# jdm365/Compression_Algorithms

Measured on AMD Instinct MI355X. Metric: encode GB/s on enwik9 at 1/2/4/8 MI355X; ratio vs ref; round-trip bit-exact, higher is better.
Workload: dtype u8; 1 GPU; deflate (LZ77 W=32 KiB len<=31 + per-block dynamic Huffman over the 286-symbol alphabet, mode H), independent 64 KiB blocks; 1000000000 enwik-shaped bytes in the job, 1000000000 on rank 0; input_seed=12345, mode=H, input_bytes_job=1000000000, input_bytes_rank0=1000000000, compressed_bytes_job=516875560, compressed_bytes_rank0=516875560, gather_to_rank0=False, parallelism=blocks sharded over 1 GPU(s), weak scaling

## Files before the change

### compression_algorithms_amd/csrc/common.h

```cpp
#pragma once

#include <hip/hip_runtime.h>
#include <stdint.h>
#include <stdio.h>
#include <string.h>

#include "../../include/mi_codec.h"
#include "lz_plan.h"

#define MI_WAVE 64

#define MI_PROF_KERNELS 48
#define MI_PROF_PENDING 8192
struct mi_prof_entry {
    const char *name;
    double      ms;
    uint64_t    launches, bytes;
};
struct mi_prof_pending { hipEvent_t a, b; uint64_t bytes; int idx; };

struct mi_ctx {
    int         device = 0;
    hipStream_t stream = nullptr;
    hipStream_t side = nullptr;
    hipStream_t fb = nullptr;
    hipStream_t fb2 = nullptr;
    hipStream_t parse = nullptr;
    hipEvent_t  ev_find[MI_SETS] = {}, ev_done[MI_SETS] = {}, ev_part[MI_SETS] = {}, ev_fb[MI_SETS] = {}, ev_replay[MI_SETS] = {}, ev_wide[MI_SETS] = {};
    hipEvent_t  ev_fork = nullptr;
    int         last_hip = 0;
    int         profiling = 0;
    int         num_cu = 256;
    int         lds_rank_ok = 0;
    int         test_break_rank = 0;
    int         test_force_fb = 0;
    int         test_small_parts = 0;
    int         test_old_partition = 0;
    uint64_t   *d_stats = nullptr;
    uint32_t   *h_order = nullptr;
    uint32_t   *d_order = nullptr;
    uint32_t    order_violations = 0;
    uint32_t    order_reported = 0;
    void       *ws = nullptr;
    size_t      ws_bytes = 0;
#ifdef MI_TEST_HOOKS
    size_t      ws_asked = 0;
    const void *test_partmap = nullptr, *test_partmap_meta = nullptr;
    uint32_t    test_partmap_nb = 0;
#endif
    void       *h_pinned = nullptr;
    size_t      h_pinned_bytes = 0;
    uint64_t   *lz_dbg = nullptr;
    uint32_t   *d_err = nullptr;
    uint32_t    err_next = 0;
#define MI_ERR_SLOTS 256
    mi_prof_entry    prof[MI_PROF_KERNELS];
    int              nprof = 0;
    mi_prof_pending *pending = nullptr;
    int              npending = 0;
    hipEvent_t      *event_pool = nullptr;
    int              npool = 0;
};

#define MI_HIP(ctx, call)                                                     \
    do {                                                                      \
        hipError_t e__ = (call);                                              \
        if (e__ != hipSuccess) {                                              \
            (ctx)->last_hip = (int)e__;                                       \
            return MI_ERR_HIP;                                                \
        }                                                                     \
    } while (0)

int mi_order_poll(mi_ctx *ctx);
mi_status mi_ws_reserve(mi_ctx *ctx, size_t bytes);
uint32_t *mi_err_slot(mi_ctx *ctx, hipStream_t s);
extern "C" mi_status mi_validate_block_table(const uint64_t *h_block_bits, uint64_t nblocks, uint64_t stream_bytes, uint32_t align_bits);
hipStream_t mi_host_stream(mi_ctx *ctx);
struct mi_prof_scope {
    mi_ctx *ctx; int idx; hipStream_t s; hipEvent_t a = nullptr, b = nullptr; uint64_t pbytes = 0;
    mi_prof_scope(mi_ctx *c, const char *name, hipStream_t st, uint64_t bytes);
    ~mi_prof_scope();
};

static inline size_t mi_align_up(size_t v, size_t a) { return (v + a - 1) / a * a; }

struct mi_carver {
    uint8_t *base; size_t limit, off = 0; bool overflow = false;
    explicit mi_carver(void *b = nullptr, size_t lim = SIZE_MAX) : base((uint8_t *)b), limit(lim) {}
    template <typename T> T *take(size_t count) {
        const size_t at = mi_align_up(off, 256);
        off = at + count * sizeof(T);
        if (off > limit) overflow = true;
        return base && !overflow ? (T *)(base + at) : nullptr;
    }
    template <typename T> void take(T *&p, size_t count) { p = take<T>(count); }
    template <typename T> static T *at(T *p, size_t i) { return p ? p + i : nullptr; }
    size_t bytes() const { return mi_align_up(off, 256); }
};
template <typename F> static inline mi_status mi_ws_carve(mi_ctx *ctx, F layout)
{
    mi_carver m;
    layout(m);
    const mi_status st = mi_ws_reserve(ctx, m.bytes());
    if (st) return st;
    mi_carver cv(ctx->ws);
    layout(cv);
    return MI_OK;
}
```

### compression_algorithms_amd/csrc/ctx.hip

```cpp
#include "common.h"
#include <stdlib.h>

__global__ __launch_bounds__(512)
static void k_lds_rank_probe(uint32_t rounds, uint32_t *__restrict__ bad)
{
    __shared__ uint32_t cnt[256 * 9];
    const uint32_t tid = threadIdx.x, lane = tid & 63u, wave = tid >> 6;
    for (uint32_t i = tid; i < 256 * 9; i += 512) cnt[i] = 0;
    __syncthreads();
    uint32_t errs = 0, x = tid * 2654435761u + blockIdx.x * 40503u + 12345u;
    for (uint32_t r = 0; r < rounds; ++r) {
        x = x * 1664525u + 1013904223u;
        const uint32_t ndig = 1u << (r % 9u);
        const uint32_t d = (blockIdx.x & 1u) ? ((x >> 16) % ndig) : (((x >> 16) % ndig) * 32u) % 256u;
        const uint32_t old = atomicAdd(&cnt[d * 9 + wave], 1u);
        for (uint32_t o = 1; o < 64; ++o) {
            const uint32_t src = (lane + o) & 63u;
            const uint32_t od = __shfl(d, src), oo = __shfl(old, src);
            if (od == d && ((src < lane) != (oo < old))) ++errs;
        }
    }
    if (errs) atomicAdd(bad, errs);
}

static int lds_rank_selfcheck(mi_ctx *c)
{
    if (getenv("MI_LZ_NO_ARANK")) return 0;
    uint32_t h = 1;
    if (hipMemset(c->d_err, 0, 4) != hipSuccess) return 0;
    hipLaunchKernelGGL(k_lds_rank_probe, dim3(64), dim3(512), 0, 0, 72u, c->d_err);
    if (hipGetLastError() != hipSuccess || hipMemcpy(&h, c->d_err, 4, hipMemcpyDeviceToHost) != hipSuccess) return 0;
    (void)hipMemset(c->d_err, 0, 4);
    return h == 0;
}

extern "C" {

const char *mi_version(void) { return "mi_codec 0.1 (gfx950)"; }

const char *mi_status_str(mi_status s)
{
    switch (s) {
    case MI_OK: return "ok";
    case MI_ERR_ARG: return "bad argument";
    case MI_ERR_HIP: return "HIP call failed";
    case MI_ERR_NOMEM: return "out of memory";
    case MI_ERR_CAPACITY: return "output buffer too small";
    case MI_ERR_EMPTY_INPUT: return "empty input (reference: ERROR: Queue is empty)";
    case MI_ERR_SINGLE_SYMBOL: return "single distinct symbol (reference: ERROR: No code for character)";
    case MI_ERR_CODE_TOO_LONG: return "Huffman code longer than 32 bits";
    case MI_ERR_CORRUPT: return "corrupt stream";
    case MI_ERR_NO_DEVICE: return "no HIP device: this library has no CPU fallback";
    case MI_ERR_TRANSPORT: return "multi-device gather: RCCL missing or an RCCL call failed";
    case MI_ERR_UNSTABLE: return "a sort came out unstable (LDS atomics not lane-ordered): encode again, the context now ranks with ballots";
    }
    return "unknown";
}

mi_status mi_ctx_create(mi_ctx **out, int device)
{
    if (!out) return MI_ERR_ARG;
    *out = nullptr;
    int count = 0;
    if (hipGetDeviceCount(&count) != hipSuccess || count <= 0 || device < 0 || device >= count)
        return MI_ERR_NO_DEVICE;
    mi_ctx *c = (mi_ctx *)calloc(1, sizeof(mi_ctx));
    if (!c) return MI_ERR_NOMEM;
    c->num_cu = 256;
    c->device = device;
    if (hipSetDevice(device) != hipSuccess) { free(c); return MI_ERR_NO_DEVICE; }
    hipDeviceProp_t prop;
    if (hipGetDeviceProperties(&prop, device) == hipSuccess) c->num_cu = prop.multiProcessorCount;
    {
        int lo = 0, hi = 0;
        (void)hipDeviceGetStreamPriorityRange(&lo, &hi);
        bool ok = hipStreamCreateWithFlags(&c->side, hipStreamNonBlocking) == hipSuccess;
        ok = ok && hipStreamCreateWithPriority(&c->fb, hipStreamNonBlocking, lo) == hipSuccess;
        ok = ok && hipStreamCreateWithPriority(&c->parse, hipStreamNonBlocking, hi) == hipSuccess;
        if (!ok) { mi_ctx_destroy(c); return MI_ERR_HIP; }
    }
    for (int i = 0; i < MI_SETS; ++i) {
        hipEventCreateWithFlags(&c->ev_replay[i], hipEventDisableTiming);
        hipEventCreateWithFlags(&c->ev_wide[i], hipEventDisableTiming);
        hipEventCreateWithFlags(&c->ev_part[i], hipEventDisableTiming);
        hipEventCreateWithFlags(&c->ev_fb[i], hipEventDisableTiming);
        hipEventCreateWithFlags(&c->ev_find[i], hipEventDisableTiming);
        hipEventCreateWithFlags(&c->ev_done[i], hipEventDisableTiming);
    }
    hipEventCreateWithFlags(&c->ev_fork, hipEventDisableTiming);
    c->h_pinned_bytes = 1 << 16;
    if (hipHostMalloc(&c->h_pinned, c->h_pinned_bytes, hipHostMallocDefault) != hipSuccess) {
        mi_ctx_destroy(c); return MI_ERR_NOMEM;
    }
    if (hipMalloc((void **)&c->d_err, MI_ERR_SLOTS * sizeof(uint32_t)) != hipSuccess) { mi_ctx_destroy(c); return MI_ERR_NOMEM; }
    if (hipHostMalloc((void **)&c->h_order, 64, hipHostMallocMapped) != hipSuccess ||
        hipHostGetDevicePointer((void **)&c->d_order, c->h_order, 0) != hipSuccess) { mi_ctx_destroy(c); return MI_ERR_NOMEM; }
    c->h_order[0] = 0; c->h_order[1] = 0; c->h_order[2] = 0;
    c->lds_rank_ok = lds_rank_selfcheck(c);
    c->test_break_rank = getenv("MI_LZ_TEST_BREAK_RANK") != nullptr;
    c->test_force_fb = getenv("MI_LZ_TEST_FORCE_FALLBACK") != nullptr;
    c->test_small_parts = getenv("MI_LZ_TEST_SMALL_PARTS") != nullptr;
    c->test_old_partition = getenv("MI_LZ_TEST_OLD_PARTITION") != nullptr;
    if (hipMalloc((void **)&c->d_stats, 64) != hipSuccess || hipMemset(c->d_stats, 0, 64) != hipSuccess) { mi_ctx_destroy(c); return MI_ERR_NOMEM; }
    *out = c;
    return MI_OK;
}

void mi_ctx_destroy(mi_ctx *c)
{
    if (!c) return;
    hipSetDevice(c->device);
    hipDeviceSynchronize();
    for (int i = 0; i < c->npending; ++i) { hipEventDestroy(c->pending[i].a); hipEventDestroy(c->pending[i].b); }
    for (int i = 0; i < c->npool; ++i) hipEventDestroy(c->event_pool[i]);
    free(c->pending); free(c->event_pool);
    if (c->ws) hipFree(c->ws);
    if (c->d_err) hipFree(c->d_err);
    if (c->d_stats) hipFree(c->d_stats);
    if (c->h_pinned) hipHostFree(c->h_pinned);
    if (c->h_order) hipHostFree(c->h_order);
    if (c->stream) hipStreamDestroy(c->stream);
    if (c->side) hipStreamDestroy(c->side);
    if (c->fb) hipStreamDestroy(c->fb);
    if (c->fb2) hipStreamDestroy(c->fb2);
    if (c->parse) hipStreamDestroy(c->parse);
    for (int i = 0; i < MI_SETS; ++i) {
        if (c->ev_replay[i]) hipEventDestroy(c->ev_replay[i]);
        if (c->ev_wide[i]) hipEventDestroy(c->ev_wide[i]);
        if (c->ev_find[i]) hipEventDestroy(c->ev_find[i]);
        if (c->ev_done[i]) hipEventDestroy(c->ev_done[i]);
        if (c->ev_part[i]) hipEventDestroy(c->ev_part[i]);
        if (c->ev_fb[i]) hipEventDestroy(c->ev_fb[i]);
    }
    if (c->ev_fork) hipEventDestroy(c->ev_fork);
    free(c);
}

int mi_last_hip_error(const mi_ctx *c) { return c ? c->last_hip : 0; }

mi_status mi_sync(mi_ctx *c, void *stream)
{
    if (!c) return MI_ERR_ARG;
    MI_HIP(c, hipStreamSynchronize((hipStream_t)stream));
    mi_order_poll(c);
    if (c->order_violations != c->order_reported) { c->order_reported = c->order_violations; return MI_ERR_UNSTABLE; }
    return MI_OK;
}

uint32_t mi_order_violations(mi_ctx *c)
{
    if (!c) return 0;
    mi_order_poll(c);
    return c->order_violations;
}

mi_status mi_lz_path_stats(mi_ctx *c, uint64_t *fallback_blocks, uint64_t *wide_parts)
{
    if (!c || !c->d_stats) return MI_ERR_ARG;
    uint64_t h[2] = {0, 0};
    MI_HIP(c, hipSetDevice(c->device));
    MI_HIP(c, hipDeviceSynchronize());
    MI_HIP(c, hipMemcpy(h, c->d_stats, 16, hipMemcpyDeviceToHost));
    if (fallback_blocks) *fallback_blocks = h[0];
    if (wide_parts) *wide_parts = h[1];
    return MI_OK;
}

mi_status mi_set_profiling(mi_ctx *c, int on)
{
    if (!c) return MI_ERR_ARG;
    if (on && !c->pending) {
        c->pending = (mi_prof_pending *)calloc(MI_PROF_PENDING, sizeof(mi_prof_pending));
        c->event_pool = (hipEvent_t *)calloc(2 * MI_PROF_PENDING, sizeof(hipEvent_t));
        if (!c->pending || !c->event_pool) { free(c->pending); free(c->event_pool); c->pending = nullptr; c->event_pool = nullptr; return MI_ERR_NOMEM; }
    }
    c->profiling = on;
    return MI_OK;
}

int mi_get_kernel_times(mi_ctx *c, mi_kernel_time *out, int cap)
{
    if (!c || !out) return 0;
    for (int i = 0; i < c->npending; ++i) {
        mi_prof_pending &q = c->pending[i];
        float ms = 0.f;
        hipEventSynchronize(q.b);
        if (hipEventElapsedTime(&ms, q.a, q.b) == hipSuccess) {
            mi_prof_entry &p = c->prof[q.idx];
            p.ms += ms; p.launches += 1; p.bytes += q.bytes;
        }
        c->event_pool[c->npool++] = q.a;
        c->event_pool[c->npool++] = q.b;
    }
    c->npending = 0;
    int n = 0;
    for (int i = 0; i < c->nprof; ++i) {
        mi_prof_entry &p = c->prof[i];
        if (!p.launches || n >= cap) continue;
        out[n].name = p.name;
        out[n].ms = p.ms / (double)p.launches;
        out[n].launches = p.launches;
        out[n].bytes = p.bytes;
        ++n;
        p.ms = 0; p.launches = 0; p.bytes = 0;
    }
    return n;
}

}

uint32_t *mi_err_slot(mi_ctx *c, hipStream_t s)
{
    uint32_t *e = c->d_err + (c->err_next++ % MI_ERR_SLOTS);
    if (hipMemsetAsync(e, 0, 4, s) != hipSuccess) return nullptr;
    return e;
}

extern "C" mi_status mi_validate_block_table(const uint64_t *t, uint64_t nblocks, uint64_t stream_bytes, uint32_t align_bits)
{
    if (!t || !align_bits) return MI_ERR_ARG;
    if (stream_bytes > (UINT64_MAX >> 3)) return MI_ERR_ARG;
    const uint64_t limit = stream_bytes * 8;
    uint64_t prev = t[0];
    if (prev % align_bits) return MI_ERR_CORRUPT;
    for (uint64_t i = 1; i <= nblocks; ++i) {
        const uint64_t v = t[i];
        if (v < prev || (v % align_bits)) return MI_ERR_CORRUPT;
        prev = v;
    }
    return prev <= limit ? MI_OK : MI_ERR_CORRUPT;
}

hipStream_t mi_host_stream(mi_ctx *c)
{
    if (!c->stream && hipStreamCreateWithFlags(&c->stream, hipStreamNonBlocking) != hipSuccess) c->stream = nullptr;
    return c->stream;
}


int mi_order_poll(mi_ctx *c)
{
    if (!c->h_order) return 0;
    const uint32_t v = __atomic_exchange_n(c->h_order, 0u, __ATOMIC_RELAXED);
    if (!v) return 0;
    ++c->order_violations;
    c->lds_rank_ok = 0;
    return 1;
}

#ifdef MI_TEST_HOOKS
#define MI_WS_GUARD 4096u
#else
#define MI_WS_GUARD 0u
#endif

mi_status mi_ws_reserve(mi_ctx *c, size_t bytes)
{
#ifdef MI_TEST_HOOKS
    if (bytes > c->ws_asked) c->ws_asked = bytes;
#endif
    if (bytes + MI_WS_GUARD <= c->ws_bytes) return MI_OK;
    MI_HIP(c, hipDeviceSynchronize());
    if (c->ws) { MI_HIP(c, hipFree(c->ws)); c->ws = nullptr; c->ws_bytes = 0; }
    size_t want = mi_align_up(bytes + bytes / 8 + MI_WS_GUARD, 1 << 20);
    if (hipMalloc(&c->ws, want) != hipSuccess) {
        (void)hipGetLastError();
        want = mi_align_up(bytes + MI_WS_GUARD, 1 << 20);
        c->ws = nullptr;
        if (hipMalloc(&c->ws, want) != hipSuccess) { (void)hipGetLastError(); c->ws = nullptr; return MI_ERR_NOMEM; }
    }
    c->ws_bytes = want;
    return MI_OK;
}

#ifdef MI_TEST_HOOKS
extern "C" int64_t mi_test_ws_guard(mi_ctx *c, int op)
{
    if (!c || op < 0 || op > 2) return -2;
    if (op == 0) { c->ws_asked = 0; return -1; }
    if (hipDeviceSynchronize() != hipSuccess) return -2;
    const size_t from = c->ws_asked < c->ws_bytes ? c->ws_asked : c->ws_bytes, len = c->ws_bytes - from;
    uint8_t *d = (uint8_t *)c->ws + from;
    if (op == 1) return !len || hipMemset(d, 0xA5, len) == hipSuccess ? -1 : -2;
    uint8_t *h = (uint8_t *)malloc(len ? len : 1);
    if (!h) return -2;
    int64_t at = -1;
    if (len && hipMemcpy(h, d, len, hipMemcpyDeviceToHost) != hipSuccess) at = -2;
    for (size_t i = 0; at == -1 && i < len; ++i) if (h[i] != 0xA5) at = (int64_t)(from + i);
    free(h);
    return at;
}
#endif

static hipEvent_t take_event(mi_ctx *c)
{
    if (c->npool > 0) return c->event_pool[--c->npool];
    hipEvent_t e = nullptr;
    hipEventCreate(&e);
    return e;
}

mi_prof_scope::mi_prof_scope(mi_ctx *c, const char *name, hipStream_t st, uint64_t bytes) : ctx(c), idx(-1), s(st)
{
    if (!c->profiling || !c->pending || c->npending >= MI_PROF_PENDING) return;
    for (int i = 0; i < c->nprof; ++i) if (strcmp(c->prof[i].name, name) == 0) { idx = i; break; }
    if (idx < 0) {
        if (c->nprof >= MI_PROF_KERNELS) return;
        idx = c->nprof++;
        c->prof[idx].name = name; c->prof[idx].ms = 0; c->prof[idx].launches = 0; c->prof[idx].bytes = 0;
    }
    a = take_event(c); b = take_event(c);
    pbytes = bytes;
    hipEventRecord(a, s);
}

mi_prof_scope::~mi_prof_scope()
{
    if (idx < 0) return;
    hipEventRecord(b, s);
    mi_prof_pending &q = ctx->pending[ctx->npending++];
    q.a = a; q.b = b; q.bytes = pbytes; q.idx = idx;
}
```

### compression_algorithms_amd/csrc/lz2_partition.hip

```cpp
#include "lz_common.h"
#include "lz2.h"
#include "internal.h"

namespace {
#define PT_TICK(k) do { if (sc.dbg && tid == 0) { long long t2 = clock64(); atomicAdd((unsigned long long *)&sc.dbg[32 + (k)], (unsigned long long)(t2 - tk)); tk = t2; } } while (0)

struct Lz2PartLds {
    uint32_t *s_grp;
    uint32_t *s_safe;
    uint64_t *s_scan64;
    uint32_t *s_scan32;
    uint32_t *s_thr;
    uint32_t *s_pstart;
    uint8_t  *s_gpart;
    uint8_t  *s_wrank;
    uint32_t *s_s0, *s_flag;
    uint32_t *s_K, *s_wbase, *s_wbase2;
};

__device__ __forceinline__ bool lz2_partition_cuts(const Lz2PartLds &L, const LzP &P, const Lz2Scratch &sc, uint32_t lb, uint32_t n, int tid, long long &tk,
                                                   uint32_t &gstart_out)
{
    uint32_t *const s_grp = L.s_grp, *const s_safe = L.s_safe, *const s_scan32 = L.s_scan32, *const s_thr = L.s_thr, *const s_pstart = L.s_pstart;
    uint64_t *const s_scan64 = L.s_scan64;
    uint8_t *const s_gpart = L.s_gpart, *const s_wrank = L.s_wrank;
    uint32_t &s_s0 = *L.s_s0, &s_flag = *L.s_flag, &s_K = *L.s_K, &s_wbase = *L.s_wbase, &s_wbase2 = *L.s_wbase2;
    const uint32_t T = 1u << P.tbits;
    const uint32_t gshift = P.tbits - LZ2_NG_BITS, Gw = 1u << gshift;

    const uint32_t g0 = tid * (LZ2_NG / 1024);
    AffMax mine{0, AM_NEG};
    for (uint32_t k = 0; k < LZ2_NG / 1024; ++k) {
        const int32_t c = (int32_t)s_grp[g0 + k];
        mine = am_then(mine, AffMax{c - (int32_t)Gw, c > 0 ? c - 1 : 0});
    }
    uint64_t tot64;
    const uint64_t pre64 = block_exclusive_scan<uint64_t>(am_pack(mine), OpAm(), am_pack(AffMax{0, AM_NEG}), s_scan64, &tot64);
    const AffMax pre = am_unpack(pre64), total = am_unpack(tot64);
    const int32_t x0 = P.deflate ? (total.b > 0 ? total.b : 0) : 0;
    {
        int32_t x = x0 + pre.a > pre.b ? x0 + pre.a : pre.b;
        if (x < 0) x = 0;
        uint32_t safe_bits = 0;
        for (uint32_t k = 0; k < LZ2_NG / 1024; ++k) {
            const int32_t c = (int32_t)s_grp[g0 + k];
            int32_t o = x + c - (int32_t)Gw;
            const int32_t o2 = c > 0 ? c - 1 : 0;
            o = o > o2 ? o : o2;
            if (o < 0) o = 0;
            if (o == 0) safe_bits |= 1u << k;
            x = o;
        }
        atomicOr(&s_safe[g0 >> 5], safe_bits << (g0 & 31u));
        if (safe_bits) atomicMin(&s_s0, g0 + (uint32_t)__builtin_ctz(safe_bits));
    }
    {
        uint32_t sum = 0;
        for (uint32_t k = 0; k < LZ2_NG / 1024; ++k) sum += s_grp[g0 + k];
        uint32_t tot;
        uint32_t run = block_exclusive_scan<uint32_t>(sum, OpAddU32(), 0u, s_scan32, &tot);
        for (uint32_t k = 0; k < LZ2_NG / 1024; ++k) { run += s_grp[g0 + k]; s_grp[g0 + k] = run; }
    }
    __syncthreads();

    PT_TICK(2);
    Lz2BlockMeta *mt = sc.meta + lb;
    const uint32_t s0 = s_s0;
    const bool no_safe = (s0 == ~0u);
    const uint32_t gstart = P.deflate ? (no_safe ? 0u : ((s0 + 1u) & (LZ2_NG - 1u))) : 0u;
    const uint32_t base = gstart << gshift;
    auto cum_incl = [&](uint32_t gr) -> uint32_t {
        const uint32_t g = (gstart + gr) & (LZ2_NG - 1u);
        const uint32_t before = gstart ? s_grp[gstart - 1] : 0u;
        return g >= gstart ? s_grp[g] - before : s_grp[g] + (n - before);
    };
    auto is_safe = [&](uint32_t gr) -> bool {
        const uint32_t g = (gstart + gr) & (LZ2_NG - 1u);
        return (s_safe[g >> 5] >> (g & 31u)) & 1u;
    };
    if (tid < 64) {
        const uint32_t lane = (uint32_t)tid;
        uint32_t k = 0, cur = 0, glo = 0;
        bool bad = false;
        if (lane == 0) s_thr[0] = 0;
        auto cut_below = [&](uint32_t limit) -> int32_t {
            const uint32_t span = (gshift <= 6u) ? (65536u >> gshift) : LZ2_NG;
            uint32_t lo = glo, hi = (glo + span < LZ2_NG) ? glo + span : LZ2_NG - 1;
            while (lo < hi) {
                const uint32_t len = hi - lo, step = (len + 63u) / 64u;
                const uint32_t pr = lo + lane * step;
                const bool over = (pr < hi) && cum_incl(pr) > limit;
                const uint64_t mk = __ballot(over);
                if (mk == 0ull) lo = lo + ((len - 1u) / step) * step + 1u;
                else {
                    const uint32_t j = (uint32_t)__builtin_ctzll(mk);
                    hi = lo + j * step;
                    if (j) lo = lo + (j - 1u) * step + 1u;
                }
            }
            for (int32_t g = (int32_t)lo - 1; g >= (int32_t)glo; g -= 64) {
                const int32_t c = g - (int32_t)lane;
                const uint64_t mk = __ballot(c >= (int32_t)glo && is_safe((uint32_t)c));
                if (mk) return g - (int32_t)__builtin_ctzll(mk);
            }
            return -1;
        };
#ifdef MI_TEST_HOOKS
        const uint32_t cap_s = (P.flags & LZP_SMALL_PARTS) ? 640u : LZ2_CAP_S;
#else
        constexpr uint32_t cap_s = LZ2_CAP_S;
#endif
        while (n - cur > cap_s) {
            int32_t gr = cut_below(cur + cap_s);
            if (gr < (int32_t)glo) {
                if (n - cur <= LZ2_CAP) break;
                gr = cut_below(cur + LZ2_CAP);
            }
            if (gr < (int32_t)glo || k + 2 > LZ2_MAXPARTS) { bad = true; break; }
            cur = cum_incl((uint32_t)gr);
            glo = (uint32_t)gr + 1u;
            ++k;
            if (lane == 0) s_thr[k] = glo << gshift;
        }
#ifdef MI_TEST_HOOKS
        if (P.flags & LZP_FORCE_FB) bad = true;
#endif
        if (lane == 0) {
            s_thr[k + 1] = T;
            s_K = k + 1;
            if (bad) s_flag = 1;
        }
    }
    __syncthreads();
    const uint32_t K = s_K;
    PT_TICK(3);
    if (tid < K) {
        const uint32_t a = s_thr[tid], b = s_thr[tid + 1];
        auto cnt_below = [&](uint32_t h) -> uint32_t {
            if (h == 0) return 0u;
            return cum_incl((h >> gshift) - 1u);
        };
        const uint32_t cnt = b > a ? cnt_below(b) - cnt_below(a) : 0u;
        s_pstart[tid] = cnt_below(a);
        if (cnt > LZ2_CAP) atomicOr(&s_flag, 1u);
        mt->part_start[tid] = cnt_below(a);
        mt->part_count[tid] = cnt;
        mt->part_lo[tid] = a;
    }
    if (tid == 0) {
        s_pstart[K] = n;
        mt->n = n; mt->nparts = K; mt->base = base;
        mt->nbig = 0; mt->nbig_entries = 0;
    }
    __syncthreads();
    if (tid == 0) {
        const bool fb = (s_flag != 0) || (P.deflate && no_safe);
        mt->fallback = fb ? 1u : 0u;
        if (fb) { const uint32_t k = atomicAdd(sc.fallback_count, 1u); sc.fallback_list[k] = lb; }
    }
    if (s_flag != 0 || (P.deflate && no_safe)) {
        if (tid == 0 && P.stats) atomicAdd((unsigned long long *)&P.stats[0], 1ull);
        return false;
    }
    {
        if (tid == 0) {
            uint32_t ns = 0, nw = 0;
            for (uint32_t k = 0; k < K; ++k) s_wrank[k] = (uint8_t)(mt->part_count[k] <= LZ2_CAP_S ? ns++ : nw++);
            s_wbase = atomicAdd(sc.work_count, ns);
            s_wbase2 = nw ? atomicAdd(sc.work_count + 1, nw) : 0u;
            if (nw && P.stats) atomicAdd((unsigned long long *)&P.stats[1], (unsigned long long)nw);
        }
        __syncthreads();
        if (tid < (int)K) {
            const uint64_t item = (uint64_t)lb | ((uint64_t)tid << 16) | ((uint64_t)mt->part_count[tid] << 24) | ((uint64_t)mt->part_start[tid] << 40);
            if (mt->part_count[tid] <= LZ2_CAP_S) sc.work[s_wbase + s_wrank[tid]] = item;
            else sc.work[sc.work_slots - 1u - (s_wbase2 + s_wrank[tid])] = item;
        }
    }

    {
        constexpr uint32_t GPT = LZ2_NG / 1024;
        const uint32_t gr0 = (uint32_t)tid * GPT;
        uint32_t lo = 0, hi = K - 1;
        { const uint32_t h = gr0 << gshift; while (lo < hi) { const uint32_t mid = (lo + hi + 1) >> 1; if (s_thr[mid] <= h) lo = mid; else hi = mid - 1; } }
        uint32_t nxt = lo + 1 < K ? s_thr[lo + 1] : 0xFFFFFFFFu;
        for (uint32_t k = 0; k < GPT; ++k) {
            const uint32_t h = (gr0 + k) << gshift;
            while (h >= nxt) { ++lo; nxt = lo + 1 < K ? s_thr[lo + 1] : 0xFFFFFFFFu; }
            s_gpart[gr0 + k] = (uint8_t)lo;
        }
    }
    __syncthreads();
    PT_TICK(4);
    gstart_out = gstart;
    return true;
}

template <bool DESC>
__global__ __launch_bounds__(1024)
void k_lz2_partition(const uint8_t *__restrict__ in, uint64_t n_total, LzP P, Lz2Scratch sc, uint64_t block0)
{
    __shared__ __attribute__((aligned(16))) uint8_t s_in[LZ_MAX_BLOCK + LZ_TAIL + 16];
    __shared__ uint32_t s_grp[LZ2_NG];
    __shared__ uint32_t s_safe[LZ2_NG / 32];
    __shared__ uint64_t s_scan64[18];
    __shared__ uint32_t s_scan32[18];
    __shared__ uint32_t s_thr[LZ2_MAXPARTS + 1];
    __shared__ uint32_t s_pstart[LZ2_MAXPARTS + 1];
    __shared__ uint32_t s_s0, s_flag, s_K, s_wbase, s_wbase2;
    __shared__ uint8_t s_wrank[LZ2_MAXPARTS];
    __shared__ __attribute__((aligned(16))) uint8_t s_gpart[LZ2_NG];

    const int tid = threadIdx.x;
    const uint32_t lb = blockIdx.x;
    long long tk = clock64();
    const uint8_t *src; uint32_t n;
    lz_block_src<DESC>(in, n_total, P.block, block0, lb, src, n);
    const uint32_t T = 1u << P.tbits, Tmask = T - 1u;
    const uint32_t gshift = P.tbits - LZ2_NG_BITS;

    lz_block_to_lds_of<DESC>(s_in, src, n, (uint32_t)tid);
    for (uint32_t i = tid; i < LZ2_NG; i += 1024) s_grp[i] = 0;
    for (uint32_t i = tid; i < LZ2_NG / 32; i += 1024) s_safe[i] = 0;
    if (tid == 0) { s_s0 = ~0u; s_flag = 0; }
    __syncthreads();
    auto home_of = [&](uint32_t p) -> uint32_t { return lz_mix32(lds_word(s_in, p)) & Tmask; };
    PT_TICK(0);
    uint32_t gcache[32];
#pragma unroll
    for (uint32_t i = 0; i < 64u; ++i) {
        const uint32_t p = (uint32_t)tid + 1024u * i;
        uint32_t g = 0;
        if (p < n) { g = home_of(p) >> gshift; atomicAdd(&s_grp[g], 1u); }
        if (i & 1u) gcache[i >> 1] |= g << 16; else gcache[i >> 1] = g;
    }
    __syncthreads();
    PT_TICK(1);

    uint32_t gstart_;
    if (!lz2_partition_cuts(Lz2PartLds{s_grp, s_safe, s_scan64, s_scan32, s_thr, s_pstart, s_gpart, s_wrank, &s_s0, &s_flag, &s_K, &s_wbase, &s_wbase2}, P, sc, lb, n, tid, tk, gstart_)) return;

    uint8_t *part_in = reinterpret_cast<uint8_t *>(s_grp);
    {
#pragma unroll
        for (uint32_t i = 0; i < 64u; ++i) {
            const uint32_t p = (uint32_t)tid + 1024u * i;
            const uint32_t g = (gcache[i >> 1] >> (16u * (i & 1u))) & 0xFFFFu;
            part_in[p] = (p < n) ? s_gpart[(g - gstart_) & (LZ2_NG - 1u)] : (uint8_t)PMP_NONE;
        }
    }
    __syncthreads();
    PT_TICK(5);
    {
        uint32_t *stage = reinterpret_cast<uint32_t *>(s_in);
        static_assert(sizeof(s_in) >= PMP_BLOCK_BYTES && LZ_MAX_BLOCK == 64u * 1024u, "the planes of a block are staged in s_in, 64 positions per thread");
        const uint4 *srcv = reinterpret_cast<const uint4 *>(part_in) + 4u * (uint32_t)tid;
        uint32_t w[16], lo[PMP_PLANES], hi[PMP_PLANES];
#pragma unroll
        for (uint32_t q = 0; q < 4u; ++q) { const uint4 v = srcv[q]; w[4 * q] = v.x; w[4 * q + 1] = v.y; w[4 * q + 2] = v.z; w[4 * q + 3] = v.w; }
        pmp_planes_of_bytes(w, lo, hi);
#pragma unroll
        for (uint32_t b = 0; b < PMP_PLANES; ++b)
            *reinterpret_cast<uint2 *>(stage + b * (PMP_PLANE_BYTES / 4u) + 2u * (uint32_t)tid) = make_uint2(lo[b], hi[b]);
        __syncthreads();
        uint4 *dst = reinterpret_cast<uint4 *>(sc.partmap + (size_t)lb * (PMP_BLOCK_BYTES / 4u));
        const uint4 *stv = reinterpret_cast<const uint4 *>(stage);
        for (uint32_t i = tid; i < PMP_BLOCK_BYTES / 16u; i += 1024u) dst[i] = stv[i];
    }
    PT_TICK(6);
    if (sc.dbg && tid == 0) atomicAdd((unsigned long long *)&sc.dbg[47], 1ull);
}

__global__ __launch_bounds__(1024, 8)
void k_lz2_partition_direct(const uint8_t *__restrict__ in, uint64_t n_total, LzP P, Lz2Scratch sc, uint64_t block0)
{
    __shared__ __attribute__((aligned(16))) uint32_t s_grp[LZ2_NG];
    __shared__ uint32_t s_safe[LZ2_NG / 32];
    __shared__ uint64_t s_scan64[18];
    __shared__ uint32_t s_scan32[18];
    __shared__ uint32_t s_thr[LZ2_MAXPARTS + 1];
    __shared__ uint32_t s_pstart[LZ2_MAXPARTS + 1];
    __shared__ uint32_t s_s0, s_flag, s_K, s_wbase, s_wbase2;
    __shared__ uint8_t s_wrank[LZ2_MAXPARTS];
    static_assert(LZ_MAX_BLOCK == 64u * 1024u, "64 positions per thread");

    const int tid = threadIdx.x;
    const uint32_t lb = blockIdx.x;
    long long tk = clock64();
    const uint8_t *src; uint32_t n;
    lz_block_src<false>(in, n_total, P.block, block0, lb, src, n);
    const uint32_t Tmask = (1u << P.tbits) - 1u;
    const uint32_t gshift = P.tbits - LZ2_NG_BITS;
    const uint32_t p0 = 64u * (uint32_t)tid;

    uint32_t w[17];
    {
        const uint32_t last = n ? (n - 1u) & ~15u : 0u;
        uint4 v[4] = {};
        uint32_t v4 = 0u;
        if (n) {
#pragma unroll
            for (uint32_t k = 0; k < 4u; ++k) { const uint32_t o = p0 + 16u * k; v[k] = *reinterpret_cast<const uint4 *>(src + (o <= last ? o : last)); }
            v4 = *reinterpret_cast<const uint32_t *>(src + (p0 + 64u <= last ? p0 + 64u : last));
        }
#pragma unroll
        for (uint32_t k = 0; k < 4u; ++k) { w[4 * k] = v[k].x; w[4 * k + 1] = v[k].y; w[4 * k + 2] = v[k].z; w[4 * k + 3] = v[k].w; }
        w[16] = v4;
    }
    for (uint32_t i = tid; i < LZ2_NG; i += 1024) s_grp[i] = 0;
    for (uint32_t i = tid; i < LZ2_NG / 32; i += 1024) s_safe[i] = 0;
    if (tid == 0) { s_s0 = ~0u; s_flag = 0; }
    __syncthreads();
    PT_TICK(0);
    if (p0 + 68u > n) {
#pragma unroll
        for (uint32_t j = 0; j < 17u; ++j) {
            const uint32_t o = p0 + 4u * j, keep = n > o ? n - o : 0u;
            if (keep < 4u) w[j] &= keep ? (1u << (8u * keep)) - 1u : 0u;
        }
    }
    auto group_of = [&](uint32_t i) -> uint32_t {
        const uint32_t word = (i & 3u) ? __builtin_amdgcn_alignbyte(w[(i >> 2) + 1], w[i >> 2], i & 3u) : w[i >> 2];
        return (lz_mix32(word) & Tmask) >> gshift;
    };
    uint32_t gcache[32];
    if (p0 < n) {
#pragma unroll
        for (uint32_t i = 0; i < 64u; ++i) {
            const uint32_t g = group_of(i);
            atomicAdd(&s_grp[g], p0 + i < n ? 1u : 0u);
            if (i & 1u) gcache[i >> 1] |= g << 16; else gcache[i >> 1] = g;
            if ((i & 7u) == 7u) __builtin_amdgcn_sched_barrier(0);
        }
    }
    __syncthreads();
    PT_TICK(1);

    uint8_t *s_gpart = reinterpret_cast<uint8_t *>(s_grp);
    uint32_t gstart_;
    if (!lz2_partition_cuts(Lz2PartLds{s_grp, s_safe, s_scan64, s_scan32, s_thr, s_pstart, s_gpart, s_wrank, &s_s0, &s_flag, &s_K, &s_wbase, &s_wbase2}, P, sc, lb, n, tid, tk, gstart_)) return;

    uint32_t pb[16], lo[PMP_PLANES], hi[PMP_PLANES];
#pragma unroll
    for (uint32_t q = 0; q < 16u; ++q) pb[q] = PMP_NONE * 0x01010101u;
    if (p0 < n) {
#pragma unroll
        for (uint32_t i = 0; i < 64u; ++i) {
            const uint32_t g = (gcache[i >> 1] >> (16u * (i & 1u))) & 0xFFFFu;
            const uint32_t look = s_gpart[(g - gstart_) & (LZ2_NG - 1u)], part = (p0 + i < n) ? look : PMP_NONE;
            if (i & 3u) pb[i >> 2] |= part << (8u * (i & 3u)); else pb[i >> 2] = part;
            if ((i & 7u) == 7u) __builtin_amdgcn_sched_barrier(0);
        }
    }
    pmp_planes_of_bytes(pb, lo, hi);
    PT_TICK(5);
    uint2 *dst = reinterpret_cast<uint2 *>(sc.partmap + (size_t)lb * (PMP_BLOCK_BYTES / 4u)) + tid;
#pragma unroll
    for (uint32_t b = 0; b < PMP_PLANES; ++b) dst[b * (PMP_PLANE_BYTES / 8u)] = make_uint2(lo[b], hi[b]);
    PT_TICK(6);
    if (sc.dbg && tid == 0) atomicAdd((unsigned long long *)&sc.dbg[47], 1ull);
}
}

void lz2_launch_partition(const uint8_t *d_in, uint64_t n, const LzP &P, const Lz2Scratch &sc, uint64_t block0, uint32_t nb, hipStream_t s)
{
    bool direct = !(P.flags & LZP_DESC) && (((uintptr_t)d_in) & 15u) == 0 && P.block % 16u == 0 && P.block <= LZ_MAX_BLOCK;
#ifdef MI_TEST_HOOKS
    if (P.flags & LZP_OLD_PARTITION) direct = false;
#endif
    if (P.flags & LZP_DESC) hipLaunchKernelGGL(k_lz2_partition<true>, dim3(nb), dim3(1024), 0, s, d_in, n, P, sc, block0);
    else if (direct) hipLaunchKernelGGL(k_lz2_partition_direct, dim3(nb), dim3(1024), 0, s, d_in, n, P, sc, block0);
    else hipLaunchKernelGGL(k_lz2_partition<false>, dim3(nb), dim3(1024), 0, s, d_in, n, P, sc, block0);
}

__global__ __launch_bounds__(1024)
void k_selftest_scan(const int32_t *__restrict__ ab, uint64_t *__restrict__ out)
{
    __shared__ uint64_t s_tmp[18];
    const int tid = threadIdx.x;
    uint64_t tot;
    const uint64_t pre = block_exclusive_scan<uint64_t>(am_pack(AffMax{ab[2 * tid], ab[2 * tid + 1]}), OpAm(), am_pack(AffMax{0, AM_NEG}), s_tmp, &tot);
    out[tid] = pre;
    if (tid == 0) out[1024] = tot;
}

extern "C" int mi_selftest_scan(mi_ctx *ctx, const int32_t *h_ab , uint64_t *h_out )
{
    if (!ctx || !h_ab || !h_out) return 0;
    int32_t *d_ab = nullptr; uint64_t *d_out = nullptr;
    if (hipMalloc(&d_ab, 2048 * 4) != hipSuccess || hipMalloc(&d_out, 1025 * 8) != hipSuccess) return 0;
    int ok = hipMemcpy(d_ab, h_ab, 2048 * 4, hipMemcpyHostToDevice) == hipSuccess;
    if (ok) { hipLaunchKernelGGL(k_selftest_scan, dim3(1), dim3(1024), 0, 0, d_ab, d_out); ok = hipDeviceSynchronize() == hipSuccess; }
    if (ok) ok = hipMemcpy(h_out, d_out, 1025 * 8, hipMemcpyDeviceToHost) == hipSuccess;
    (void)hipFree(d_ab); (void)hipFree(d_out);
    return ok;
}
```

### compression_algorithms_amd/csrc/lz_common.h

```cpp
#pragma once
#include "common.h"
#include "lz_plan.h"
#include <type_traits>

#define LZ_MAX_BLOCK   65536u
#define LZ_TAIL        64u
#define LZ_NONE16      0xFFFFu

#define LZ_TILE_NOM    4096u
#define LZ_TILE_CAP    8192u
#define LZ_GIANT_MIN   (LZ_TILE_CAP - LZ_TILE_NOM)
#define LZ_GIANT_CAP   18432u
#define LZ_MAX_TILES   (LZ_MAX_BLOCK / LZ_TILE_NOM)
#define LZ_WAVE_MIN    128u
#define LZ_MAX_GIANTS_PER_BLOCK (LZ_MAX_BLOCK / LZ_WAVE_MIN + 32u)
#ifndef LZ_TILE_WAVE_MIN
#define LZ_TILE_WAVE_MIN 16u
#endif

struct LzP {
    uint32_t wbits, lbits, tbits, deflate, block;
    uint32_t flags;
    uint32_t *order_flag;
    uint64_t *stats;
};
#define LZP_ARANK 1u
#define LZP_BREAK 2u
#define LZP_FORCE_FB 4u
#define LZP_DESC 8u
#define LZP_LAZY 16u
#define LZP_SMALL_PARTS 32u
#define LZP_OLD_PARTITION 64u

__device__ __forceinline__ void lz_order_violation(const LzP &P)
{
    if (P.order_flag) __hip_atomic_fetch_or(P.order_flag, 1u, __ATOMIC_RELAXED, __HIP_MEMORY_SCOPE_SYSTEM);
}

static inline LzP lz_params_of(mi_ctx *ctx, const mi_lz_params *p)
{
    mi_order_poll(ctx);
    uint32_t fl = ctx->lds_rank_ok ? LZP_ARANK : 0u;
    if (fl && ctx->test_break_rank) fl |= LZP_BREAK;
    if (ctx->test_force_fb) fl |= LZP_FORCE_FB;
    if (ctx->test_small_parts) fl |= LZP_SMALL_PARTS;
    if (ctx->test_old_partition) fl |= LZP_OLD_PARTITION;
    if (p->parse == MI_PARSE_LAZY) fl |= LZP_LAZY;
    return LzP{p->wbits, p->lbits, p->tbits, p->deflate, p->block, fl, ctx->d_order, ctx->d_stats};
}

struct LzBlkDesc {
    const uint8_t *src;
    uint32_t n;
    uint32_t item;
    uint32_t blk;
    uint16_t last;
    uint16_t skip;
};
static_assert(sizeof(LzBlkDesc) == 24, "the table's stride");
#define LZ_DESC_PAD 0xFFFFFFFFu

template <bool DESC>
__device__ __forceinline__ void lz_block_src(const uint8_t *__restrict__ in, uint64_t n_total, uint32_t block, uint64_t block0, uint32_t lb,
                                             const uint8_t *&src, uint32_t &n)
{
    if constexpr (DESC) {
        const LzBlkDesc *d = reinterpret_cast<const LzBlkDesc *>(in) + (block0 + lb);
        src = d->src; n = d->n;
    } else {
        const uint64_t off = (block0 + lb) * (uint64_t)block;
        n = (uint32_t)((n_total - off) < block ? (n_total - off) : block);
        src = in + off;
    }
}

template <bool DICT>
__device__ __forceinline__ uint32_t lz_block_skip(const uint8_t *__restrict__ in, uint64_t block0, uint32_t lb)
{
    if constexpr (DICT) return reinterpret_cast<const LzBlkDesc *>(in)[block0 + lb].skip;
    else return 0u;
}

struct LzBlockMeta {
    uint32_t n;
    uint32_t ngroups;
    uint32_t anom_idx;
    uint32_t limit_idx;
    uint32_t rot;
    uint32_t pad[3];
};

__device__ __forceinline__ uint64_t lz_pack(uint32_t gid, uint32_t pos, uint32_t rloc, uint32_t pid)
{
    return (uint64_t)gid | ((uint64_t)pos << 16) | ((uint64_t)rloc << 32) | ((uint64_t)pid << 48);
}

struct LzScratch {
    uint16_t    *posA, *posB;
    uint64_t    *eA, *eB;
    uint16_t    *cand;
    LzBlockMeta *meta;
    uint32_t    *giant_count;
    uint32_t    *giant_list;
    uint32_t     giant_cap;
    uint32_t    *slot;
    uint64_t    *block_bits;
};
#define LZ_SLOT_WORDS  (LZ_MAX_BLOCK / 2 + 16)
#define LZ_DEFH_HIST_AT 32000u

struct LzwScratch {
    uint64_t *eA, *eB;
    uint32_t *gid;
    uint32_t *rd;
    uint32_t *cstart;
    uint32_t *ncl;
    uint8_t  *t_live;
    uint32_t *t_pos, *t_mix;
    uint32_t *slot_of;
    uint32_t *cand;
    uint32_t *ent;
    uint32_t *relw;
    uint16_t *cand_e;
    uint64_t *clist[6];
    uint32_t *ccount;
    uint32_t *slot;
    uint64_t *block_bits;
    uint32_t  S, slot_words;
};

__device__ __forceinline__ uint32_t lz_giant_slot(const LzScratch &sc, uint32_t g, uint32_t n_back)
{
    return g < n_back ? sc.giant_cap - 1u - g : g - n_back;
}

__device__ __forceinline__ uint32_t lz_mix32(uint32_t w)
{
    uint32_t k = w * 0xcc9e2d51u;
    k = (k << 15) | (k >> 17);
    k *= 0x1b873593u;
    uint32_t h = (k << 13) | (k >> 19);
    h = h * 5u + 0xe6546b64u;
    h ^= h >> 16; h *= 0x85ebca6bu;
    h ^= h >> 13; h *= 0xc2b2ae35u;
    h ^= h >> 16;
    return h;
}

__device__ __forceinline__ uint32_t lds_word(const uint8_t *s, uint32_t p)
{
    const uint32_t *a = reinterpret_cast<const uint32_t *>(s + (p & ~3u));
    const uint64_t v = (uint64_t)a[0] | ((uint64_t)a[1] << 32);
    return (uint32_t)(v >> ((p & 3u) * 8u));
}

__device__ __forceinline__ void lz_block_to_lds(uint8_t *s_dst, const uint8_t *__restrict__ src, uint32_t n, uint32_t tid)
{
    constexpr uint32_t NIT = (LZ_MAX_BLOCK + LZ_TAIL + 1024u * 16u - 1u) / (1024u * 16u);
    const bool vec_ok = ((((uintptr_t)src) & 15u) == 0) && n >= 16u;
    if (vec_ok) {
        const uint32_t last = (n - 16u) & ~15u;
        uint4 v[NIT];
#pragma unroll
        for (uint32_t k = 0; k < NIT; ++k) {
            const uint32_t i = tid * 16u + k * 1024u * 16u;
            v[k] = *reinterpret_cast<const uint4 *>(src + (i <= last ? i : last));
        }
#pragma unroll
        for (uint32_t k = 0; k < NIT; ++k) {
            const uint32_t i = tid * 16u + k * 1024u * 16u;
            if (i >= LZ_MAX_BLOCK + LZ_TAIL) continue;
            if (i + 16u <= n) *reinterpret_cast<uint4 *>(s_dst + i) = v[k];
            else if (i >= n) *reinterpret_cast<uint4 *>(s_dst + i) = make_uint4(0u, 0u, 0u, 0u);
            else {
#pragma unroll 1
                for (uint32_t b = 0; b < 16; ++b) s_dst[i + b] = (i + b < n) ? src[i + b] : (uint8_t)0;
            }
        }
    } else {
#pragma unroll 1
        for (uint32_t i = tid * 16u; i < LZ_MAX_BLOCK + LZ_TAIL; i += 1024u * 16u) {
#pragma unroll 1
            for (uint32_t b = 0; b < 16; ++b) s_dst[i + b] = (i + b < n) ? src[i + b] : (uint8_t)0;
        }
    }
}

struct LzVec2 { uint4 lo, hi; };
__device__ __forceinline__ LzVec2 lz_load16_pair(const uint8_t *__restrict__ src, uint32_t n, uint32_t i)
{
    const uintptr_t a = (uintptr_t)(src + i);
    const uint32_t sh = (uint32_t)(a & 15u);
    const uint4 *lo = reinterpret_cast<const uint4 *>(a - sh);
    const uint32_t want = (n - i) < 16u ? (n - i) : 16u;
    LzVec2 v;
    v.lo = lo[0];
    v.hi = lo[sh + want > 16u ? 1 : 0];
    return v;
}
__device__ __forceinline__ uint4 lz_shift16(const LzVec2 &v, uint32_t sh , uint32_t valid )
{
    const uint32_t w[8] = {v.lo.x, v.lo.y, v.lo.z, v.lo.w, v.hi.x, v.hi.y, v.hi.z, v.hi.w};
    const uint32_t ws = sh >> 2, bs = (sh & 3u) * 8u;
    uint32_t e[5], o[4];
#pragma unroll
    for (uint32_t k = 0; k < 5u; ++k) e[k] = ws == 0u ? w[k] : ws == 1u ? w[k + 1] : ws == 2u ? w[k + 2] : w[k + 3];
#pragma unroll
    for (uint32_t k = 0; k < 4u; ++k) {
        o[k] = (uint32_t)((((uint64_t)e[k + 1] << 32) | e[k]) >> bs);
        const uint32_t keep = valid > 4u * k ? valid - 4u * k : 0u;
        if (keep < 4u) o[k] &= keep ? (1u << (8u * keep)) - 1u : 0u;
    }
    return make_uint4(o[0], o[1], o[2], o[3]);
}
__device__ __forceinline__ void lz_block_to_lds_any(uint8_t *s_dst, const uint8_t *__restrict__ src, uint32_t n, uint32_t tid)
{
    constexpr uint32_t NIT = (LZ_MAX_BLOCK + LZ_TAIL + 1024u * 16u - 1u) / (1024u * 16u);
    const uint32_t sh = (uint32_t)((uintptr_t)src & 15u);
    const uint32_t last = n ? (n - 1u) & ~15u : 0u;
    LzVec2 v[NIT];
    if (n) {
#pragma unroll
        for (uint32_t k = 0; k < NIT; ++k) {
            const uint32_t i = tid * 16u + k * 1024u * 16u;
            v[k] = lz_load16_pair(src, n, i <= last ? i : last);
        }
    }
#pragma unroll
    for (uint32_t k = 0; k < NIT; ++k) {
        const uint32_t i = tid * 16u + k * 1024u * 16u;
        if (i >= LZ_MAX_BLOCK + LZ_TAIL) continue;
        if (i >= n) *reinterpret_cast<uint4 *>(s_dst + i) = make_uint4(0u, 0u, 0u, 0u);
        else *reinterpret_cast<uint4 *>(s_dst + i) = lz_shift16(v[k], sh, (n - i) < 16u ? (n - i) : 16u);
    }
}
__device__ __forceinline__ void lz_chunk64_any(const uint8_t *__restrict__ src, uint32_t n, uint32_t p0, uint4 (&v4)[4])
{
    const uint32_t sh = (uint32_t)((uintptr_t)src & 15u), last = (n - 1u) & ~15u;
    LzVec2 v[4];
#pragma unroll
    for (uint32_t k = 0; k < 4u; ++k) { const uint32_t i = p0 + 16u * k; v[k] = lz_load16_pair(src, n, i <= last ? i : last); }
#pragma unroll
    for (uint32_t k = 0; k < 4u; ++k) {
        const uint32_t i = p0 + 16u * k;
        v4[k] = lz_shift16(v[k], sh, i >= n ? 0u : (n - i) < 16u ? (n - i) : 16u);
    }
}
template <bool DESC>
__device__ __forceinline__ void lz_block_to_lds_of(uint8_t *s_dst, const uint8_t *__restrict__ src, uint32_t n, uint32_t tid)
{
    if constexpr (DESC) lz_block_to_lds_any(s_dst, src, n, tid);
    else lz_block_to_lds(s_dst, src, n, tid);
}

template <int CTRL, int ROW_MASK, typename T>
__device__ __forceinline__ T dpp_move(T v, T old)
{
    static_assert(sizeof(T) % 4 == 0, "32-bit words");
    uint32_t w[sizeof(T) / 4], o[sizeof(T) / 4];
    __builtin_memcpy(w, &v, sizeof(T));
    __builtin_memcpy(o, &old, sizeof(T));
#pragma unroll
    for (unsigned k = 0; k < sizeof(T) / 4; ++k)
        w[k] = (uint32_t)__builtin_amdgcn_update_dpp((int)o[k], (int)w[k], CTRL, ROW_MASK, 0xF, false);
    T r;
    __builtin_memcpy(&r, w, sizeof(T));
    return r;
}

template <typename T, typename Op>
__device__ __forceinline__ T wave_inclusive_scan(T v, Op op, T ident)
{
    v = op(dpp_move<0x111, 0xF>(v, ident), v);
    v = op(dpp_move<0x112, 0xF>(v, ident), v);
    v = op(dpp_move<0x114, 0xF>(v, ident), v);
    v = op(dpp_move<0x118, 0xF>(v, ident), v);
    v = op(dpp_move<0x142, 0xA>(v, ident), v);
    v = op(dpp_move<0x143, 0xC>(v, ident), v);
    return v;
}

template <typename T, typename Op>
__device__ __forceinline__ T block_exclusive_scan(T v, Op op, T ident, T *s_tmp, T *total)
{
    const int lane = threadIdx.x & 63, wave = threadIdx.x >> 6, nw = (blockDim.x + 63) >> 6;
    T inc = wave_inclusive_scan(v, op, ident);
    T exc = dpp_move<0x138, 0xF>(inc, ident);
    if (lane == 63) s_tmp[wave] = inc;
    __syncthreads();
    if (threadIdx.x == 0) {
        T run = ident;
        for (int w = 0; w < nw; ++w) { T t = s_tmp[w]; s_tmp[w] = run; run = op(run, t); }
        s_tmp[nw] = run;
    }
    __syncthreads();
    T res = op(s_tmp[wave], exc);
    *total = s_tmp[nw];
    __syncthreads();
    return res;
}

struct OpAddU32 { __device__ uint32_t operator()(uint32_t a, uint32_t b) const { return a + b; } };
struct OpMaxI32 { __device__ int32_t operator()(int32_t a, int32_t b) const { return a > b ? a : b; } };

struct AffMax { int32_t a, b; };
__device__ __forceinline__ uint64_t am_pack(AffMax f) { return ((uint64_t)(uint32_t)f.a << 32) | (uint32_t)f.b; }
__device__ __forceinline__ AffMax am_unpack(uint64_t v) { AffMax f; f.a = (int32_t)(v >> 32); f.b = (int32_t)(uint32_t)v; return f; }
#define AM_NEG (-(1 << 28))
__device__ __forceinline__ AffMax am_then(AffMax first, AffMax second)
{
    AffMax r;
    r.a = first.a + second.a;
    if (r.a < AM_NEG) r.a = AM_NEG;
    int32_t t = first.b + second.a;
    if (t < AM_NEG) t = AM_NEG;
    r.b = t > second.b ? t : second.b;
    return r;
}
struct OpAm { __device__ uint64_t operator()(uint64_t earlier, uint64_t later) const { return am_pack(am_then(am_unpack(earlier), am_unpack(later))); } };

struct RadixNoHook { __device__ __forceinline__ void operator()(uint32_t, uint32_t) const {} };
__device__ __forceinline__ uint32_t radix_cnt_add(uint32_t *cnt, uint32_t i, uint32_t v) { return atomicAdd(&cnt[i], v); }
__device__ __forceinline__ uint32_t radix_cnt_add(uint16_t *cnt, uint32_t i, uint32_t v)
{
    const uint32_t sh = 16u * (i & 1u);
    return (atomicAdd(reinterpret_cast<uint32_t *>(cnt) + (i >> 1), v << sh) >> sh) & 0xFFFFu;
}
template <int NWAVES> __device__ __forceinline__ uint32_t radix_seg(uint32_t n) { return ((n + (uint32_t)(NWAVES * 64) - 1u) / (uint32_t)(NWAVES * 64)) * 64u; }
template <int D, bool SKIP = false> struct RadixDepth { static constexpr int value = D; static constexpr bool skip_identity = SKIP; };
template <int NWAVES, int NBITS, typename E, typename CntRow, typename Load, typename Digit, typename Store, typename Hook = RadixNoHook, typename Depth = RadixDepth<1>>
__device__ __forceinline__ bool radix_pass(uint32_t n, CntRow *s_cnt, Load load, Digit digit, Store store, uint32_t arank = 0u , uint64_t *dbg = nullptr,
                                           bool counted = false, Hook hook = Hook(), Depth = Depth())
{
    long long tk_ = dbg ? clock64() : 0;
#define RP_TICK(k) do { if (dbg && threadIdx.x == 0) { long long t2 = clock64(); atomicAdd((unsigned long long *)&dbg[k], (unsigned long long)(t2 - tk_)); tk_ = t2; } } while (0)
    using C = std::remove_reference_t<decltype(s_cnt[0][0])>;
    static_assert(std::is_same<C, uint32_t>::value || std::is_same<C, uint16_t>::value, "32- or 16-bit counters");
    static_assert(sizeof(CntRow) / sizeof(C) >= (1u << NBITS), "counter row too narrow for the digit");
    constexpr int ND = 1 << NBITS;
    constexpr int NT = NWAVES * 64;
    constexpr int ST = NWAVES + 1;
    C *cnt = &s_cnt[0][0];
    const int tid = threadIdx.x, lane = tid & 63, wave = tid >> 6;
    const uint32_t seg = ((n + (uint32_t)NT - 1u) / (uint32_t)NT) * 64u;
    const uint32_t a = wave * seg, b = (a + seg < n) ? a + seg : n;
    if (!counted) {
        for (int i = tid; i < ND * ST; i += NT) cnt[i] = 0;
        __syncthreads();
        if constexpr (Depth::value > 1) {
// ... 147 lines not shown
```

Before: 26.43 GB/s.

## Replace binary-search part cuts with ballot-based coarse index and single-window scan

The single-wave partition walker now precomputes cumulative counts at 64-group strides into registers. Each cut is found with a ballot/popcount over those checkpoints followed by one 64-wide window scan, replacing the iterative multi-step binary search. The cut position's cumulative value is returned directly so it is not recomputed. The walker wave gets raised scheduling priority, the part map is written as packed 16-byte LDS stores, and the old cut path is kept behind a test flag. This targets the serial latency of the partition walk, at the cost of more code and register use.

Result: faster. 26.73 GB/s, median of 6 (+1.1%).

```diff
diff --git a/compression_algorithms_amd/csrc/common.h b/compression_algorithms_amd/csrc/common.h
--- a/compression_algorithms_amd/csrc/common.h
+++ b/compression_algorithms_amd/csrc/common.h
@@ -36,6 +36,7 @@
     int         test_force_fb = 0;
     int         test_small_parts = 0;
     int         test_old_partition = 0;
+    int         test_old_cuts = 0;
     uint64_t   *d_stats = nullptr;
     uint32_t   *h_order = nullptr;
     uint32_t   *d_order = nullptr;
diff --git a/compression_algorithms_amd/csrc/ctx.hip b/compression_algorithms_amd/csrc/ctx.hip
--- a/compression_algorithms_amd/csrc/ctx.hip
+++ b/compression_algorithms_amd/csrc/ctx.hip
@@ -101,6 +101,7 @@
     c->test_force_fb = getenv("MI_LZ_TEST_FORCE_FALLBACK") != nullptr;
     c->test_small_parts = getenv("MI_LZ_TEST_SMALL_PARTS") != nullptr;
     c->test_old_partition = getenv("MI_LZ_TEST_OLD_PARTITION") != nullptr;
+    c->test_old_cuts = getenv("MI_LZ_TEST_OLD_CUTS") != nullptr;
     if (hipMalloc((void **)&c->d_stats, 64) != hipSuccess || hipMemset(c->d_stats, 0, 64) != hipSuccess) { mi_ctx_destroy(c); return MI_ERR_NOMEM; }
     *out = c;
     return MI_OK;
diff --git a/compression_algorithms_amd/csrc/lz2_partition.hip b/compression_algorithms_amd/csrc/lz2_partition.hip
--- a/compression_algorithms_amd/csrc/lz2_partition.hip
+++ b/compression_algorithms_amd/csrc/lz2_partition.hip
@@ -28,9 +28,11 @@
     const uint32_t T = 1u << P.tbits;
     const uint32_t gshift = P.tbits - LZ2_NG_BITS, Gw = 1u << gshift;
 
-    const uint32_t g0 = tid * (LZ2_NG / 1024);
+    constexpr uint32_t GPT = LZ2_NG / 1024;
+    static_assert(GPT == 16u, "a thread's part bytes are one 16-byte word");
+    const uint32_t g0 = tid * GPT;
     AffMax mine{0, AM_NEG};
-    for (uint32_t k = 0; k < LZ2_NG / 1024; ++k) {
+    for (uint32_t k = 0; k < GPT; ++k) {
         const int32_t c = (int32_t)s_grp[g0 + k];
         mine = am_then(mine, AffMax{c - (int32_t)Gw, c > 0 ? c - 1 : 0});
     }
@@ -42,7 +44,7 @@
         int32_t x = x0 + pre.a > pre.b ? x0 + pre.a : pre.b;
         if (x < 0) x = 0;
         uint32_t safe_bits = 0;
-        for (uint32_t k = 0; k < LZ2_NG / 1024; ++k) {
+        for (uint32_t k = 0; k < GPT; ++k) {
             const int32_t c = (int32_t)s_grp[g0 + k];
             int32_t o = x + c - (int32_t)Gw;
             const int32_t o2 = c > 0 ? c - 1 : 0;
@@ -56,35 +58,66 @@
     }
     {
         uint32_t sum = 0;
-        for (uint32_t k = 0; k < LZ2_NG / 1024; ++k) sum += s_grp[g0 + k];
+        for (uint32_t k = 0; k < GPT; ++k) sum += s_grp[g0 + k];
         uint32_t tot;
         uint32_t run = block_exclusive_scan<uint32_t>(sum, OpAddU32(), 0u, s_scan32, &tot);
-        for (uint32_t k = 0; k < LZ2_NG / 1024; ++k) { run += s_grp[g0 + k]; s_grp[g0 + k] = run; }
+        for (uint32_t k = 0; k < GPT; ++k) { run += s_grp[g0 + k]; s_grp[g0 + k] = run; }
     }
     __syncthreads();
 
     PT_TICK(2);
     Lz2BlockMeta *mt = sc.meta + lb;
-    const uint32_t s0 = s_s0;
+    const uint32_t s0 = (uint32_t)__builtin_amdgcn_readfirstlane((int)s_s0);
     const bool no_safe = (s0 == ~0u);
     const uint32_t gstart = P.deflate ? (no_safe ? 0u : ((s0 + 1u) & (LZ2_NG - 1u))) : 0u;
     const uint32_t base = gstart << gshift;
+    const uint32_t before = gstart ? (uint32_t)__builtin_amdgcn_readfirstlane((int)s_grp[gstart - 1]) : 0u;
     auto cum_incl = [&](uint32_t gr) -> uint32_t {
         const uint32_t g = (gstart + gr) & (LZ2_NG - 1u);
-        const uint32_t before = gstart ? s_grp[gstart - 1] : 0u;
         return g >= gstart ? s_grp[g] - before : s_grp[g] + (n - before);
     };
     auto is_safe = [&](uint32_t gr) -> bool {
         const uint32_t g = (gstart + gr) & (LZ2_NG - 1u);
         return (s_safe[g >> 5] >> (g & 31u)) & 1u;
     };
+    const bool walker = __builtin_amdgcn_readfirstlane(tid) < 64;
+    if (walker) __builtin_amdgcn_s_setprio(3);
     if (tid < 64) {
         const uint32_t lane = (uint32_t)tid;
         uint32_t k = 0, cur = 0, glo = 0;
         bool bad = false;
         if (lane == 0) s_thr[0] = 0;
-        auto cut_below = [&](uint32_t limit) -> int32_t {
-            const uint32_t span = (gshift <= 6u) ? (65536u >> gshift) : LZ2_NG;
+        const uint32_t span = (gshift <= 6u) ? (65536u >> gshift) : LZ2_NG;
+        uint32_t cp[4];
+#pragma unroll
+        for (uint32_t q = 0; q < 4u; ++q) cp[q] = cum_incl(64u * (lane + 64u * q) + 63u);
+        auto cut_below = [&](uint32_t limit, uint32_t &upto) -> int32_t {
+            uint32_t j = 0;
+#pragma unroll
+            for (uint32_t q = 0; q < 4u; ++q) j += (uint32_t)__popcll(__ballot(cp[q] <= limit));
+            const uint32_t hi0 = (glo + span < LZ2_NG) ? glo + span : LZ2_NG - 1, hi = hi0 < 64u * j + 64u ? hi0 : 64u * j + 64u;
+            const int32_t w0 = (int32_t)hi - 64, c = w0 + (int32_t)lane;
+            const bool on = c >= (int32_t)glo;
+            const uint32_t g = (gstart + (uint32_t)c) & (LZ2_NG - 1u);
+            uint32_t cum = 0u, sw = 0u;
+            if (on) { cum = s_grp[g]; sw = s_safe[g >> 5]; }
+            cum = g >= gstart ? cum - before : cum + (n - before);
+            const uint64_t mo = __ballot(on && cum > limit);
+            const uint64_t ms = __ballot(on && ((sw >> (g & 31u)) & 1u)) & (mo ? (1ull << __builtin_ctzll(mo)) - 1ull : ~0ull);
+            if (ms) {
+                const uint32_t l = 63u - (uint32_t)__builtin_clzll(ms);
+                upto = (uint32_t)__builtin_amdgcn_readlane((int)cum, (int)l);
+                return w0 + (int32_t)l;
+            }
+            for (int32_t gb = w0 - 1; gb >= (int32_t)glo; gb -= 64) {
+                const int32_t cb = gb - (int32_t)lane;
+                const uint64_t mk = __ballot(cb >= (int32_t)glo && is_safe((uint32_t)cb));
+                if (mk) { const int32_t gr = gb - (int32_t)__builtin_ctzll(mk); upto = cum_incl((uint32_t)gr); return gr; }
+            }
+            return -1;
+        };
+#ifdef MI_TEST_HOOKS
+        auto cut_below_old = [&](uint32_t limit, uint32_t &upto) -> int32_t {
             uint32_t lo = glo, hi = (glo + span < LZ2_NG) ? glo + span : LZ2_NG - 1;
             while (lo < hi) {
                 const uint32_t len = hi - lo, step = (len + 63u) / 64u;
@@ -101,23 +134,29 @@
             for (int32_t g = (int32_t)lo - 1; g >= (int32_t)glo; g -= 64) {
                 const int32_t c = g - (int32_t)lane;
                 const uint64_t mk = __ballot(c >= (int32_t)glo && is_safe((uint32_t)c));
-                if (mk) return g - (int32_t)__builtin_ctzll(mk);
+                if (mk) { const int32_t gr = g - (int32_t)__builtin_ctzll(mk); upto = cum_incl((uint32_t)gr); return gr; }
             }
             return -1;
         };
+        const bool old_cuts = (P.flags & LZP_OLD_CUTS) != 0u;
+        auto cut = [&](uint32_t limit, uint32_t &upto) -> int32_t { return old_cuts ? cut_below_old(limit, upto) : cut_below(limit, upto); };
+#else
+        auto cut = cut_below;
+#endif
 #ifdef MI_TEST_HOOKS
         const uint32_t cap_s = (P.flags & LZP_SMALL_PARTS) ? 640u : LZ2_CAP_S;
 #else
         constexpr uint32_t cap_s = LZ2_CAP_S;
 #endif
         while (n - cur > cap_s) {
-            int32_t gr = cut_below(cur + cap_s);
+            uint32_t upto = 0u;
+            int32_t gr = cut(cur + cap_s, upto);
             if (gr < (int32_t)glo) {
                 if (n - cur <= LZ2_CAP) break;
-                gr = cut_below(cur + LZ2_CAP);
+                gr = cut(cur + LZ2_CAP, upto);
             }
             if (gr < (int32_t)glo || k + 2 > LZ2_MAXPARTS) { bad = true; break; }
-            cur = cum_incl((uint32_t)gr);
+            cur = upto;
             glo = (uint32_t)gr + 1u;
             ++k;
             if (lane == 0) s_thr[k] = glo << gshift;
@@ -131,6 +170,7 @@
             if (bad) s_flag = 1;
         }
     }
+    if (walker) __builtin_amdgcn_s_setprio(0);
     __syncthreads();
     const uint32_t K = s_K;
     PT_TICK(3);
@@ -179,16 +219,18 @@
     }
 
     {
-        constexpr uint32_t GPT = LZ2_NG / 1024;
         const uint32_t gr0 = (uint32_t)tid * GPT;
         uint32_t lo = 0, hi = K - 1;
         { const uint32_t h = gr0 << gshift; while (lo < hi) { const uint32_t mid = (lo + hi + 1) >> 1; if (s_thr[mid] <= h) lo = mid; else hi = mid - 1; } }
         uint32_t nxt = lo + 1 < K ? s_thr[lo + 1] : 0xFFFFFFFFu;
+        uint32_t pk[GPT / 4u];
+#pragma unroll
         for (uint32_t k = 0; k < GPT; ++k) {
             const uint32_t h = (gr0 + k) << gshift;
             while (h >= nxt) { ++lo; nxt = lo + 1 < K ? s_thr[lo + 1] : 0xFFFFFFFFu; }
-            s_gpart[gr0 + k] = (uint8_t)lo;
-        }
+            if (k & 3u) pk[k >> 2] |= lo << (8u * (k & 3u)); else pk[k >> 2] = lo;
+        }
+        *reinterpret_cast<uint4 *>(s_gpart + gr0) = make_uint4(pk[0], pk[1], pk[2], pk[3]);
     }
     __syncthreads();
     PT_TICK(4);
@@ -201,7 +243,7 @@
 void k_lz2_partition(const uint8_t *__restrict__ in, uint64_t n_total, LzP P, Lz2Scratch sc, uint64_t block0)
 {
     __shared__ __attribute__((aligned(16))) uint8_t s_in[LZ_MAX_BLOCK + LZ_TAIL + 16];
-    __shared__ uint32_t s_grp[LZ2_NG];
+    __shared__ __attribute__((aligned(16))) uint32_t s_grp[LZ2_NG];
     __shared__ uint32_t s_safe[LZ2_NG / 32];
     __shared__ uint64_t s_scan64[18];
     __shared__ uint32_t s_scan32[18];
diff --git a/compression_algorithms_amd/csrc/lz_common.h b/compression_algorithms_amd/csrc/lz_common.h
--- a/compression_algorithms_amd/csrc/lz_common.h
+++ b/compression_algorithms_amd/csrc/lz_common.h
@@ -31,6 +31,7 @@
 #define LZP_LAZY 16u
 #define LZP_SMALL_PARTS 32u
 #define LZP_OLD_PARTITION 64u
+#define LZP_OLD_CUTS 128u
 
 __device__ __forceinline__ void lz_order_violation(const LzP &P)
 {
@@ -45,6 +46,7 @@
     if (ctx->test_force_fb) fl |= LZP_FORCE_FB;
     if (ctx->test_small_parts) fl |= LZP_SMALL_PARTS;
     if (ctx->test_old_partition) fl |= LZP_OLD_PARTITION;
+    if (ctx->test_old_cuts) fl |= LZP_OLD_CUTS;
     if (p->parse == MI_PARSE_LAZY) fl |= LZP_LAZY;
     return LzP{p->wbits, p->lbits, p->tbits, p->deflate, p->block, fl, ctx->d_order, ctx->d_stats};
 }
```
